# DSXiangLi/ChineseNER

Hardware: NVIDIA H100
Metric: sentences/sec bert_bilstm_crf MSRA L=128 (higher is better)
Workload: dtype bf16

## Files before the change

chinesener_b200/csrc/gemm_tc.cu:

```cuda
#include <stdlib.h>

#include <mutex>

#include "tc_common.cuh"

namespace {

using namespace tc;

constexpr int BM = 128;
constexpr int BK = 64;
constexpr int MMA_K = 16;
constexpr int NUM_MMA_WG = 2;
constexpr float kSkFixupCost = 10.0f;
constexpr int NUM_THREADS = 128 * (1 + NUM_MMA_WG);

constexpr int OUT_CHUNK_BYTES = 64 * 128;
constexpr int OUT_STAGE_BYTES = NUM_MMA_WG * 2 * OUT_CHUNK_BYTES;

template <int BN>
struct Cfg {
  static constexpr int STAGES = (BN == 256 || BN == 192) ? 4 : ((BN == 128) ? 6 : 8);
  static constexpr int A_BYTES = BM * BK * 2;
  static constexpr int B_BYTES = BN * BK * 2;
  static constexpr int RING_BYTES = STAGES * (A_BYTES + B_BYTES);
  static constexpr size_t SMEM = (size_t)RING_BYTES + OUT_STAGE_BYTES + 256;
  static_assert(SMEM <= 227 * 1024, "shared memory per block");
};

struct EpiArgs {
  const float* bias;
  const float* residual;
};

template <int EPI>
__host__ __device__ constexpr bool epi_f32() { return EPI == NER_EPI_F32 || EPI == NER_EPI_RES_F32 || EPI == NER_EPI_RES_RELU_F32; }

__device__ __forceinline__ float gelu_tanh(float x) {
  const float u = 0.7978845608028654f * fmaf(0.044715f * x * x, x, x);
  const float hx = 0.5f * x;
  return fmaf(hx, tanh_approx(u), hx);
}
__device__ __forceinline__ float gelu_erf(float x) { return 0.5f * x * (1.f + erff(x * 0.7071067811865476f)); }

__device__ __forceinline__ uint32_t pack_bf16x2(float a, float b) {
  __nv_bfloat162 v = __floats2bfloat162_rn(a, b);
  return *reinterpret_cast<uint32_t*>(&v);
}

struct SkArgs {
  float4* ws;
  int* flags;
};

struct SegIter {
  int num_kb, num_tiles, tile, stride;
  long long u, u1;
  bool sk;
  __device__ SegIter(bool sk_, int num_tiles_, int num_kb_, int id, int count)
      : num_kb(num_kb_), num_tiles(num_tiles_), sk(sk_) {
    if (sk) {
      const long long U = (long long)num_tiles * num_kb;
      u = (long long)id * U / count;
      u1 = (long long)(id + 1) * U / count;
    } else {
      tile = id;
      stride = count;
    }
  }
  __device__ bool next(int& t, int& kb0, int& kb1) {
    if (sk) {
      if (u >= u1) return false;
      t = (int)(u / num_kb);
      kb0 = (int)(u - (long long)t * num_kb);
      const long long rem = u1 - u;
      kb1 = (rem < (long long)(num_kb - kb0)) ? kb0 + (int)rem : num_kb;
      u += kb1 - kb0;
      return true;
    }
    if (tile >= num_tiles) return false;
    t = tile;
    kb0 = 0;
    kb1 = num_kb;
    tile += stride;
    return true;
  }
};

__device__ __forceinline__ int ld_acquire_gpu(const int* p) {
  int v;
  asm volatile("ld.acquire.gpu.global.s32 %0, [%1];" : "=r"(v) : "l"(p) : "memory");
  return v;
}
__device__ __forceinline__ void st_release_gpu(int* p, int v) {
  asm volatile("st.release.gpu.global.s32 [%0], %1;" ::"l"(p), "r"(v) : "memory");
}

__device__ __forceinline__ void mma_bar_sync() {
  asm volatile("bar.sync 1, %0;" ::"n"(128 * NUM_MMA_WG) : "memory");
}

template <int BN>
struct Ring {
  uint8_t* a;
  uint8_t* b;
  uint8_t* out;
  uint64_t* full;
  uint64_t* empty;
  __device__ Ring(uint8_t* smem) {
    using C = Cfg<BN>;
    a = smem;
    b = smem + C::STAGES * C::A_BYTES;
    out = smem + C::RING_BYTES;
    full = reinterpret_cast<uint64_t*>(out + OUT_STAGE_BYTES);
    empty = full + C::STAGES;
  }
};

struct RingPos {
  int stage = 0;
  uint32_t phase = 0;
  template <int STAGES>
  __device__ __forceinline__ void advance() {
    if (++stage == STAGES) {
      stage = 0;
      phase ^= 1u;
    }
  }
};

template <int BN, int STAGES, int CL, int TA, int TB, typename DA, typename DB>
__device__ __forceinline__ void mma_kblocks(float (&acc)[BN / 2], const Ring<BN>& ring, RingPos& pos, int kb0, int kb1,
                                            uint32_t a_off, DA desc_a, DB desc_b, const uint32_t (&empty_peer)[STAGES]) {
  const int lane = threadIdx.x & 31;
  int prev = -1;
  for (int kb = kb0; kb < kb1; ++kb) {
    mbar_wait(&ring.full[pos.stage], pos.phase);
    const uint32_t a_addr = smem_u32(ring.a + pos.stage * (BM * BK * 2)) + a_off;
    const uint32_t b_addr = smem_u32(ring.b + pos.stage * (BN * BK * 2));
    reg_fence(acc);
    wgmma_fence();
#pragma unroll
    for (int k = 0; k < BK / MMA_K; ++k)
      wgmma_bf16<BN, TA, TB>(acc, desc_a(a_addr, k), desc_b(b_addr, k), (kb > kb0 || k > 0) ? 1u : 0u);
    wgmma_commit();
    reg_fence(acc);
    if (prev >= 0) {
      wgmma_wait<1>();
      reg_fence(acc);
      if (lane == 0) {
        mbar_arrive(&ring.empty[prev]);
        if constexpr (CL == 2) mbar_arrive_cluster(empty_peer[prev]);
      }
    }
    prev = pos.stage;
    pos.template advance<STAGES>();
  }
  wgmma_wait<0>();
  reg_fence(acc);
  if (lane == 0 && prev >= 0) {
    mbar_arrive(&ring.empty[prev]);
    if constexpr (CL == 2) mbar_arrive_cluster(empty_peer[prev]);
  }
}

template <int EPI>
__device__ __forceinline__ float epi_act(float v) {
  if constexpr (EPI == NER_EPI_GELU_TANH_BF16) return gelu_tanh(v);
  else if constexpr (EPI == NER_EPI_GELU_ERF_BF16) return gelu_erf(v);
  else if constexpr (EPI == NER_EPI_RELU_BF16 || EPI == NER_EPI_RES_RELU_F32) return fmaxf(v, 0.f);
  else return v;
}

__device__ __forceinline__ void wg_bar_sync(int id) {
  asm volatile("bar.sync %0, 128;" ::"r"(id) : "memory");
}

template <int BN, int EPI>
__device__ __forceinline__ void epilogue_tma(const float (&acc)[BN / 2], const EpiArgs& ep, const CUtensorMap* tma_out,
                                             uint8_t* stage, uint32_t& buf, int row_wg, int n0, int M, int N) {
  constexpr bool F32 = epi_f32<EPI>();
  constexpr bool RES = EPI == NER_EPI_RES_F32 || EPI == NER_EPI_RES_RELU_F32;
  constexpr int CW = F32 ? 32 : 64;
  constexpr int JPC = CW / 8;
  const int t = threadIdx.x & 127, lane = t & 31, warp = t >> 5;
  const int bar = 1 + (threadIdx.x >> 7);
  const int r0 = 16 * warp + (lane >> 2);
  if (row_wg >= M) return;
#pragma unroll
  for (int c = 0; c < BN / CW; ++c) {
    const int col0 = n0 + c * CW;
    if (col0 >= N) break;
    uint8_t* sb = stage + buf * OUT_CHUNK_BYTES;
    if (t == 0) tma_store_wait_read<1>();
    wg_bar_sync(bar);
    float2 b[JPC];
#pragma unroll
    for (int jj = 0; jj < JPC; ++jj) {
      const int col = col0 + 8 * jj + 2 * (lane & 3);
      b[jj] = (ep.bias != nullptr && col < N) ? __ldg(reinterpret_cast<const float2*>(ep.bias + col)) : make_float2(0.f, 0.f);
    }
    if constexpr (F32) {
#pragma unroll
      for (int jj = 0; jj < JPC; ++jj) {
        const int j = c * JPC + jj, col = col0 + 8 * jj + 2 * (lane & 3);
#pragma unroll
        for (int h = 0; h < 2; ++h) {
          const int r = r0 + 8 * h;
          float v0 = acc[4 * j + 2 * h] + b[jj].x, v1 = acc[4 * j + 2 * h + 1] + b[jj].y;
          if constexpr (RES) {
            const int row = row_wg + r;
            if (row < M && col < N) {
              const float2 rv = *reinterpret_cast<const float2*>(ep.residual + (size_t)row * N + col);
              v0 += rv.x;
              v1 += rv.y;
            }
          }
          v0 = epi_act<EPI>(v0);
          v1 = epi_act<EPI>(v1);
          const int unit = (2 * jj + ((lane & 3) >> 1)) ^ (r & 7);
          *reinterpret_cast<float2*>(sb + r * 128 + unit * 16 + 8 * (lane & 1)) = make_float2(v0, v1);
        }
      }
    } else {
      const int i = lane >> 3, r = 16 * warp + 8 * (i & 1) + (lane & 7);
      const uint32_t row_addr = smem_u32(sb) + r * 128;
#pragma unroll
      for (int jj = 0; jj < JPC; jj += 2) {
        const int j = c * JPC + jj;
        uint32_t p[4];
#pragma unroll
        for (int q = 0; q < 4; ++q) {
          const int jq = j + (q >> 1), h = q & 1;
          const float2 bq = b[jj + (q >> 1)];
          p[q] = pack_bf16x2(epi_act<EPI>(acc[4 * jq + 2 * h] + bq.x), epi_act<EPI>(acc[4 * jq + 2 * h + 1] + bq.y));
        }
        stmatrix_x4(row_addr + (((jj + (i >> 1)) ^ (r & 7)) << 4), p[0], p[1], p[2], p[3]);
      }
    }
    fence_proxy_async();
    wg_bar_sync(bar);
    if (t == 0) {
      tma_store_2d(tma_out, sb, col0, row_wg);
      tma_store_commit();
    }
    buf ^= 1u;
  }
}

template <int BN>
__device__ __forceinline__ void epilogue_accumulate(const float (&acc)[BN / 2], float* dw, int row_w, int n0, int M,
                                                    int N) {
  const int lane = threadIdx.x & 31;
#pragma unroll
  for (int j = 0; j < BN / 8; ++j) {
    const int col = n0 + 8 * j + 2 * (lane & 3);
    if (col >= N) continue;
#pragma unroll
    for (int h = 0; h < 2; ++h) {
      const int row = row_w + (lane >> 2) + 8 * h;
      if (row >= M) continue;
      float2* p = reinterpret_cast<float2*>(dw + (size_t)row * N + col);
      const float2 r = *p;
      *p = make_float2(acc[4 * j + 2 * h] + 0.f + r.x, acc[4 * j + 2 * h + 1] + 0.f + r.y);
    }
  }
}

template <int BN, int CL>
__device__ __forceinline__ void init_ring(const Ring<BN>& ring) {
  if (threadIdx.x == 0) {
    for (int s = 0; s < Cfg<BN>::STAGES; ++s) {
      mbar_init(&ring.full[s], 1);
      mbar_init(&ring.empty[s], 4 * NUM_MMA_WG * CL);
    }
    fence_barrier_init();
  }
}

template <int BN, bool SK, int CL, int EPI>
__global__ void __launch_bounds__(NUM_THREADS, 1)
gemm_bf16_tc_kernel(const __grid_constant__ CUtensorMap tma_a, const __grid_constant__ CUtensorMap tma_b,
                    const __grid_constant__ CUtensorMap tma_out, EpiArgs ep, int M, int N, int K, SkArgs skargs) {
  using C = Cfg<BN>;
  constexpr int STAGES = C::STAGES;
  nerdev::pdl_launch_dependents();

  extern __shared__ __align__(1024) uint8_t smem_raw[];
  if ((smem_u32(smem_raw) & 1023u) != 0u) __trap();
  const Ring<BN> ring(smem_raw);

  const int wg = threadIdx.x >> 7;
  const uint32_t rank = CL == 2 ? cluster_ctarank() : 0u;
  const int id = CL == 2 ? (int)(blockIdx.x >> 1) : (int)blockIdx.x;
  const int count = CL == 2 ? (int)(gridDim.x >> 1) : (int)gridDim.x;

  const int num_m = (M + CL * BM - 1) / (CL * BM);
  const int num_n = (N + BN - 1) / BN;
  const int num_tiles = num_m * num_n;
  const int num_kb = (K + BK - 1) / BK;

  if (threadIdx.x == 0) {
    tma_prefetch_desc(&tma_a);
    tma_prefetch_desc(&tma_b);
    tma_prefetch_desc(&tma_out);
  }
  init_ring<BN, CL>(ring);
  if constexpr (CL == 2) cluster_sync_all();
  else __syncthreads();
  nerdev::pdl_wait();

  if (wg == 0) {
    setmaxnreg_dec<40>();
    if (threadIdx.x < 32 && elect_one()) {
      RingPos pos;
      SegIter it(SK, num_tiles, num_kb, id, count);
      int tile, kb0, kb1;
      while (it.next(tile, kb0, kb1)) {
        const int m_blk = tile / num_n, n_blk = tile - m_blk * num_n;
        const int row_a = (m_blk * CL + (int)rank) * BM;
        for (int kb = kb0; kb < kb1; ++kb) {
          mbar_wait(&ring.empty[pos.stage], pos.phase ^ 1u);
          mbar_arrive_expect_tx(&ring.full[pos.stage], C::A_BYTES + C::B_BYTES);
          tma_load_2d(ring.a + pos.stage * C::A_BYTES, &tma_a, &ring.full[pos.stage], kb * BK, row_a);
          if constexpr (CL == 2)
            tma_load_2d_mc(ring.b + pos.stage * C::B_BYTES + rank * (C::B_BYTES / 2), &tma_b, &ring.full[pos.stage],
                           kb * BK, n_blk * BN + (int)rank * (BN / 2), (uint16_t)0x3);
          else
            tma_load_2d(ring.b + pos.stage * C::B_BYTES, &tma_b, &ring.full[pos.stage], kb * BK, n_blk * BN);
          pos.advance<STAGES>();
        }
      }
    }
  } else {
    setmaxnreg_inc<232>();
    const int mw = wg - 1;
    const int ctid = threadIdx.x - 128;
    uint8_t* stage = ring.out + mw * 2 * OUT_CHUNK_BYTES;
    uint32_t buf = 0;
    uint32_t empty_peer[STAGES];
#pragma unroll
    for (int s = 0; s < STAGES; ++s) empty_peer[s] = CL == 2 ? mapa_u32(smem_u32(&ring.empty[s]), rank ^ 1u) : 0u;
    auto da = [](uint32_t addr, int k) { return make_wgmma_desc_sw128(addr + k * MMA_K * 2); };
    constexpr size_t SLOT = (size_t)BN * BM / 2;
    float2* ws = reinterpret_cast<float2*>(skargs.ws);
    RingPos pos;
    SegIter it(SK, num_tiles, num_kb, id, count);
    int tile, kb0, kb1;
    float acc[BN / 2];
    while (it.next(tile, kb0, kb1)) {
      const int m_blk = tile / num_n, n_blk = tile - m_blk * num_n;
      const int row0 = (m_blk * CL + (int)rank) * BM;
      mma_kblocks<BN, STAGES, CL, 0, 0>(acc, ring, pos, kb0, kb1, (uint32_t)(mw * 64 * BK * 2), da, da, empty_peer);
      if (SK && kb0 > 0) {
        float2* p = ws + (size_t)blockIdx.x * SLOT + ctid;
#pragma unroll
        for (int i = 0; i < BN / 4; ++i) __stcg(p + (size_t)i * 256, make_float2(acc[2 * i], acc[2 * i + 1]));
        __threadfence();
        mma_bar_sync();
        if (ctid == 0) st_release_gpu(skargs.flags + blockIdx.x, 1);
        continue;
      }
      int c_first = 0, n_part = 0;
      if (SK && kb1 < num_kb) {
        const long long U = (long long)num_tiles * num_kb, tile_end = (long long)(tile + 1) * num_kb;
        c_first = blockIdx.x + 1;
        for (int c = c_first; c < (int)gridDim.x; ++c) {
          const long long c0 = (long long)c * U / gridDim.x, c1 = (long long)(c + 1) * U / gridDim.x;
          if (c0 >= tile_end) break;
          if (c1 > c0) ++n_part; else if (n_part == 0) ++c_first;
        }
        if (ctid == 0) {
          for (int c = 0; c < n_part; ++c) {
            unsigned spins = 0;
            while (ld_acquire_gpu(skargs.flags + c_first + c) == 0)
              if (++spins > (1u << 28)) __trap();
          }
        }
        mma_bar_sync();
        __threadfence();
        for (int c = 0; c < n_part; ++c) {
          const float2* p = ws + (size_t)(c_first + c) * SLOT + ctid;
#pragma unroll
          for (int i = 0; i < BN / 4; ++i) {
            const float2 v = __ldcg(p + (size_t)i * 256);
            acc[2 * i] += v.x;
            acc[2 * i + 1] += v.y;
          }
        }
      }
      if constexpr (EPI == NER_EPI_DIAG_DISCARD) {
        if (M < 0) {
#pragma unroll
          for (int i = 0; i < BN / 2; ++i) reinterpret_cast<float*>(ring.a)[i * 256 + ctid] = acc[i];
        }
      } else {
        epilogue_tma<BN, EPI>(acc, ep, &tma_out, stage, buf, row0 + mw * 64, n_blk * BN, M, N);
      }
      if (n_part > 0) {
        mma_bar_sync();
        if (ctid < 32)
          for (int c = ctid; c < n_part; c += 32) skargs.flags[c_first + c] = 0;
      }
    }
    if ((threadIdx.x & 127) == 0) tma_store_wait_all();
  }
  if constexpr (CL == 2) cluster_sync_all();
}

constexpr int WG_MAXP = 6;
constexpr int WG_BN = 256;

struct WgradGroup {
  CUtensorMap a[WG_MAXP], b[WG_MAXP];
  float* dw[WG_MAXP];
  int m[WG_MAXP], n[WG_MAXP], b_col0[WG_MAXP];
  int tile_start[WG_MAXP + 1];
  int count, rows;
};

__global__ void __launch_bounds__(NUM_THREADS, 1)
gemm_wgrad_group_kernel(const __grid_constant__ WgradGroup grp) {
  constexpr int BN = WG_BN;
  using C = Cfg<BN>;
  constexpr int STAGES = C::STAGES;
  constexpr int BOX = 64 * 64 * 2;
  nerdev::pdl_launch_dependents();

  extern __shared__ __align__(1024) uint8_t smem_raw[];
  if ((smem_u32(smem_raw) & 1023u) != 0u) __trap();
  const Ring<BN> ring(smem_raw);

  const int wg = threadIdx.x >> 7;
  const int num_tiles = grp.tile_start[grp.count];
  const int num_kb = (grp.rows + BK - 1) / BK;

  init_ring<BN, 1>(ring);
  __syncthreads();
  nerdev::pdl_wait();

  auto locate = [&](int tile, int& p, int& m_blk, int& n_blk) {
    p = 0;
    while (p + 1 < grp.count && tile >= grp.tile_start[p + 1]) ++p;
    const int t = tile - grp.tile_start[p], num_n = grp.n[p] / BN;
    m_blk = t / num_n;
    n_blk = t - m_blk * num_n;
  };

  if (wg == 0) {
    setmaxnreg_dec<40>();
    if (threadIdx.x < 32 && elect_one()) {
      RingPos pos;
      for (int tile = blockIdx.x; tile < num_tiles; tile += gridDim.x) {
        int p, m_blk, n_blk;
        locate(tile, p, m_blk, n_blk);
        for (int kb = 0; kb < num_kb; ++kb) {
          mbar_wait(&ring.empty[pos.stage], pos.phase ^ 1u);
          mbar_arrive_expect_tx(&ring.full[pos.stage], C::A_BYTES + C::B_BYTES);
#pragma unroll
          for (int i = 0; i < BM / 64; ++i)
            tma_load_2d(ring.a + pos.stage * C::A_BYTES + i * BOX, &grp.a[p], &ring.full[pos.stage], m_blk * BM + i * 64, kb * BK);
#pragma unroll
          for (int i = 0; i < BN / 64; ++i)
            tma_load_2d(ring.b + pos.stage * C::B_BYTES + i * BOX, &grp.b[p], &ring.full[pos.stage],
                        grp.b_col0[p] + n_blk * BN + i * 64, kb * BK);
          pos.advance<STAGES>();
        }
      }
    }
  } else {
    setmaxnreg_inc<232>();
    const int mw = wg - 1;
    const int row_in_tile = mw * 64 + ((threadIdx.x >> 5) & 3) * 16;
    const uint32_t no_peer[STAGES] = {};
    auto da = [](uint32_t addr, int k) { return make_wgmma_desc_sw128(addr + k * 2048); };
    auto db = [](uint32_t addr, int k) { return make_wgmma_desc_sw128(addr + k * 2048, BOX); };
    RingPos pos;
    float acc[BN / 2];
    for (int tile = blockIdx.x; tile < num_tiles; tile += gridDim.x) {
      int p, m_blk, n_blk;
      locate(tile, p, m_blk, n_blk);
      mma_kblocks<BN, STAGES, 1, 1, 1>(acc, ring, pos, 0, num_kb, (uint32_t)(mw * BOX), da, db, no_peer);
      epilogue_accumulate<BN>(acc, grp.dw[p], m_blk * BM + row_in_tile, n_blk * BN, grp.m[p], grp.n[p]);
    }
  }
}

constexpr int FP8_BN = 128;
constexpr int FP8_BK = 128;
constexpr int FP8_MMA_K = 32;

template <int EPI>
__host__ __device__ constexpr bool epi_e4m3() { return EPI == NER_EPI_GELU_TANH_E4M3 || EPI == NER_EPI_GELU_ERF_E4M3; }

__device__ __forceinline__ void fp8_issue(float (&t)[FP8_BN / 2], const Ring<FP8_BN>& ring, int stage, uint32_t a_off) {
  const uint32_t a_addr = smem_u32(ring.a + stage * Cfg<FP8_BN>::A_BYTES) + a_off;
  const uint32_t b_addr = smem_u32(ring.b + stage * Cfg<FP8_BN>::B_BYTES);
  reg_fence(t);
  wgmma_fence();
#pragma unroll
  for (int k = 0; k < FP8_BK / FP8_MMA_K; ++k)
    wgmma_m64n128k32_e4m3(t, make_wgmma_desc_sw128(a_addr + k * FP8_MMA_K), make_wgmma_desc_sw128(b_addr + k * FP8_MMA_K),
                          k > 0 ? 1u : 0u);
  wgmma_commit();
  reg_fence(t);
}

__device__ __forceinline__ void fp8_promote(float (&acc)[FP8_BN / 2], const float (&t)[FP8_BN / 2], float s0, float s1) {
#pragma unroll
  for (int i = 0; i < FP8_BN / 2; ++i) acc[i] = fmaf(t[i], (i & 2) ? s1 : s0, acc[i]);
}

template <int EPI>
__device__ __forceinline__ void epilogue_e4m3(float (&acc)[FP8_BN / 2], const float* bias, float* out_scale,
                                              const CUtensorMap* tma_out, uint8_t* stage, uint32_t& buf, int row_wg, int n0,
                                              int M, int N) {
  const int t = threadIdx.x & 127, lane = t & 31, warp = t >> 5;
  const int bar = 1 + (threadIdx.x >> 7);
  const int r0 = 16 * warp + (lane >> 2);
  if (row_wg >= M) return;
  uint8_t* sb = stage + buf * OUT_CHUNK_BYTES;
  if (t == 0) tma_store_wait_read<1>();
  wg_bar_sync(bar);
  float amax[2] = {0.f, 0.f};
#pragma unroll
  for (int j = 0; j < FP8_BN / 8; ++j) {
    const int col = n0 + 8 * j + 2 * (lane & 3);
    const float2 b = bias != nullptr ? __ldg(reinterpret_cast<const float2*>(bias + col)) : make_float2(0.f, 0.f);
#pragma unroll
    for (int h = 0; h < 2; ++h) {
#pragma unroll
      for (int c = 0; c < 2; ++c) {
        const float x = acc[4 * j + 2 * h + c] + (c ? b.y : b.x);
        float v;
        if constexpr (EPI == NER_EPI_GELU_ERF_E4M3) v = gelu_erf(x);
        else v = 0.5f * x * (1.f + tanhf(0.7978845608028654f * fmaf(0.044715f * x * x, x, x)));
        acc[4 * j + 2 * h + c] = v;
        amax[h] = fmaxf(amax[h], fabsf(v));
      }
    }
  }
  float inv[2];
#pragma unroll
  for (int h = 0; h < 2; ++h) {
    amax[h] = fmaxf(amax[h], __shfl_xor_sync(0xffffffffu, amax[h], 1));
    amax[h] = fmaxf(amax[h], __shfl_xor_sync(0xffffffffu, amax[h], 2));
    const float s = nerdev::e4m3_scale(amax[h]);
    inv[h] = __frcp_rn(s);
    const int row = row_wg + r0 + 8 * h;
    if ((lane & 3) == 0 && row < M) out_scale[(size_t)row * (N / FP8_BN) + n0 / FP8_BN] = s;
  }
#pragma unroll
  for (int j = 0; j < FP8_BN / 8; ++j) {
#pragma unroll
    for (int h = 0; h < 2; ++h) {
      const int r = r0 + 8 * h;
      const uint16_t q = nerdev::cvt_e4m3x2(acc[4 * j + 2 * h] * inv[h], acc[4 * j + 2 * h + 1] * inv[h]);
      *reinterpret_cast<uint16_t*>(sb + r * 128 + (((j >> 1) ^ (r & 7)) << 4) + 8 * (j & 1) + 2 * (lane & 3)) = q;
    }
  }
  fence_proxy_async();
  wg_bar_sync(bar);
  if (t == 0) {
    tma_store_2d(tma_out, sb, n0, row_wg);
    tma_store_commit();
  }
  buf ^= 1u;
}

template <int EPI>
__global__ void __launch_bounds__(NUM_THREADS, 1)
gemm_e4m3_tc_kernel(const __grid_constant__ CUtensorMap tma_a, const __grid_constant__ CUtensorMap tma_b,
                    const __grid_constant__ CUtensorMap tma_out, const float* __restrict__ a_scale,
                    const float* __restrict__ w_scale, const float* __restrict__ bias, float* __restrict__ out_scale, int M,
                    int N, int K) {
  using C = Cfg<FP8_BN>;
  constexpr int STAGES = C::STAGES;
  nerdev::pdl_launch_dependents();

  extern __shared__ __align__(1024) uint8_t smem_raw[];
  if ((smem_u32(smem_raw) & 1023u) != 0u) __trap();
  const Ring<FP8_BN> ring(smem_raw);

  const int wg = threadIdx.x >> 7;
  const int num_n = N / FP8_BN;
  const int num_tiles = ((M + BM - 1) / BM) * num_n;
  const int num_kb = K / FP8_BK;

  if (threadIdx.x == 0) {
    tma_prefetch_desc(&tma_a);
    tma_prefetch_desc(&tma_b);
    tma_prefetch_desc(&tma_out);
  }
  init_ring<FP8_BN, 1>(ring);
  __syncthreads();
  nerdev::pdl_wait();

  if (wg == 0) {
    setmaxnreg_dec<40>();
    if (threadIdx.x < 32 && elect_one()) {
      RingPos pos;
      for (int tile = blockIdx.x; tile < num_tiles; tile += gridDim.x) {
        const int m_blk = tile / num_n, n_blk = tile - m_blk * num_n;
        for (int kb = 0; kb < num_kb; ++kb) {
          mbar_wait(&ring.empty[pos.stage], pos.phase ^ 1u);
          mbar_arrive_expect_tx(&ring.full[pos.stage], C::A_BYTES + C::B_BYTES);
          tma_load_2d(ring.a + pos.stage * C::A_BYTES, &tma_a, &ring.full[pos.stage], kb * FP8_BK, m_blk * BM);
          tma_load_2d(ring.b + pos.stage * C::B_BYTES, &tma_b, &ring.full[pos.stage], kb * FP8_BK, n_blk * FP8_BN);
          pos.advance<STAGES>();
        }
      }
    }
  } else {
    setmaxnreg_inc<232>();
    const int mw = wg - 1;
    const int lane = threadIdx.x & 31, warp = (threadIdx.x >> 5) & 3;
    uint8_t* stage = ring.out + mw * 2 * OUT_CHUNK_BYTES;
    uint32_t buf = 0;
    const uint32_t a_off = (uint32_t)(mw * 64 * FP8_BK);
    RingPos pos;
    float acc[FP8_BN / 2], tmp[FP8_BN / 2];
    for (int tile = blockIdx.x; tile < num_tiles; tile += gridDim.x) {
      const int m_blk = tile / num_n, n_blk = tile - m_blk * num_n;
      const int row_wg = m_blk * BM + mw * 64, n0 = n_blk * FP8_BN;
      const int ra = row_wg + 16 * warp + (lane >> 2);
      const float* sa0 = a_scale + (size_t)min(ra, M - 1) * num_kb;
      const float* sa1 = a_scale + (size_t)min(ra + 8, M - 1) * num_kb;
#pragma unroll
      for (int i = 0; i < FP8_BN / 2; ++i) acc[i] = 0.f;
      for (int kb = 0; kb < num_kb; ++kb) {
        const float s0 = __ldg(sa0 + kb), s1 = __ldg(sa1 + kb);
        mbar_wait(&ring.full[pos.stage], pos.phase);
        fp8_issue(tmp, ring, pos.stage, a_off);
        wgmma_wait<0>();
        reg_fence(tmp);
        if (lane == 0) mbar_arrive(&ring.empty[pos.stage]);
        fp8_promote(acc, tmp, s0, s1);
        pos.advance<STAGES>();
      }
#pragma unroll
      for (int j = 0; j < FP8_BN / 8; ++j) {
        const float2 sw = __ldg(reinterpret_cast<const float2*>(w_scale + n0 + 8 * j + 2 * (lane & 3)));
        acc[4 * j] *= sw.x;
        acc[4 * j + 1] *= sw.y;
        acc[4 * j + 2] *= sw.x;
        acc[4 * j + 3] *= sw.y;
      }
      if constexpr (epi_e4m3<EPI>())
        epilogue_e4m3<EPI>(acc, bias, out_scale, &tma_out, stage, buf, row_wg, n0, M, N);
      else
        epilogue_tma<FP8_BN, NER_EPI_BF16>(acc, EpiArgs{bias, nullptr}, &tma_out, stage, buf, row_wg, n0, M, N);
    }
    if ((threadIdx.x & 127) == 0) tma_store_wait_all();
  }
}

int make_map_2d(CUtensorMap* map, const void* ptr, uint64_t rows, uint64_t cols, uint32_t box_rows, bool f32 = false) {
  EncodeTiledFn fn = tensor_map_encode_fn();
  if (fn == nullptr) return NER_ERR_NO_DRIVER;
  const uint32_t esz = f32 ? 4 : 2;
  cuuint64_t dims[2] = {cols, rows};
  cuuint64_t strides[1] = {cols * esz};
  cuuint32_t box[2] = {128 / esz, box_rows};
  cuuint32_t estr[2] = {1, 1};
  CUresult r = fn(map, f32 ? CU_TENSOR_MAP_DATA_TYPE_FLOAT32 : CU_TENSOR_MAP_DATA_TYPE_BFLOAT16, 2, const_cast<void*>(ptr),
                  dims, strides, box, estr, CU_TENSOR_MAP_INTERLEAVE_NONE, CU_TENSOR_MAP_SWIZZLE_128B,
                  CU_TENSOR_MAP_L2_PROMOTION_L2_256B, CU_TENSOR_MAP_FLOAT_OOB_FILL_NONE);
  return r == CUDA_SUCCESS ? NER_OK : NER_ERR_INVALID_ARG;
}

int gemm_auto_policy() {
  static int v = -1;
  if (v < 0) {
    const char* e = getenv("NER_GEMM_POLICY");
    v = e ? atoi(e) : 0;
  }
  return v;
}

int sm_count() { return ner_num_sms(); }

struct SkScratch {
  int dev;
  cudaStream_t st;
  float4* ws;
  int* flags;
};
constexpr int kMaxSkScratch = 16;
SkScratch g_sk[kMaxSkScratch];
int g_sk_n = 0;
std::mutex g_sk_mu;

bool sk_scratch(cudaStream_t st, SkArgs* out) {
  int dev = 0;
  if (cudaGetDevice(&dev) != cudaSuccess) return false;
  std::lock_guard<std::mutex> lk(g_sk_mu);
  for (int i = 0; i < g_sk_n; ++i)
    if (g_sk[i].dev == dev && g_sk[i].st == st) {
      out->ws = g_sk[i].ws;
      out->flags = g_sk[i].flags;
      return true;
    }
  if (g_sk_n == kMaxSkScratch) return false;
  cudaStreamCaptureStatus cap = cudaStreamCaptureStatusNone;
  if (cudaStreamIsCapturing(st, &cap) != cudaSuccess || cap != cudaStreamCaptureStatusNone) {
    (void)cudaGetLastError();
    return false;
  }
  const size_t slot = (size_t)(256 / 32) * 8 * 128 * sizeof(float4);
  float4* ws = nullptr;
  int* flags = nullptr;
  if (cudaMalloc(&ws, slot * sm_count()) != cudaSuccess) {
    (void)cudaGetLastError();
    return false;
  }
  if (cudaMalloc(&flags, sizeof(int) * sm_count()) != cudaSuccess || cudaMemset(flags, 0, sizeof(int) * sm_count()) != cudaSuccess) {
    (void)cudaGetLastError();
    cudaFree(ws);
    return false;
  }
  cudaDeviceSynchronize();
  g_sk[g_sk_n++] = SkScratch{dev, st, ws, flags};
  out->ws = ws;
  out->flags = flags;
  return true;
}

template <typename... KArgs, typename... Args>
cudaError_t launch_ex(void (*kern)(KArgs...), int grid, size_t smem, cudaStream_t st, int cl, Args... args) {
  cudaError_t e = cudaFuncSetAttribute(kern, cudaFuncAttributeMaxDynamicSharedMemorySize, (int)smem);
  if (e != cudaSuccess) return e;
  cudaLaunchConfig_t cfg{};
  cfg.gridDim = dim3(grid);
  cfg.blockDim = dim3(NUM_THREADS);
  cfg.dynamicSmemBytes = smem;
  cfg.stream = st;
  cudaLaunchAttribute attr[2];
  attr[0].id = cudaLaunchAttributeProgrammaticStreamSerialization;
  attr[0].val.programmaticStreamSerializationAllowed = 1;
  attr[1].id = cudaLaunchAttributeClusterDimension;
  attr[1].val.clusterDim.x = cl;
  attr[1].val.clusterDim.y = 1;
  attr[1].val.clusterDim.z = 1;
  cfg.attrs = attr;
  cfg.numAttrs = 2;
  return cudaLaunchKernelEx(&cfg, kern, static_cast<KArgs>(args)...);
}

template <int BN, int CL, int EPI>
int launch_gemm(const void* A, const void* Wt, EpiArgs ep, void* out, int M, int N, int K, cudaStream_t st, bool sk) {
  CUtensorMap ma, mb, mo;
  int rc = make_map_2d(&ma, A, (uint64_t)M, (uint64_t)K, BM);
  if (rc != NER_OK) return rc;
  rc = make_map_2d(&mb, Wt, (uint64_t)N, (uint64_t)K, BN / CL);
  if (rc != NER_OK) return rc;
  rc = make_map_2d(&mo, out, (uint64_t)M, (uint64_t)N, 64, epi_f32<EPI>());
  if (rc != NER_OK) return rc;
  const size_t smem = Cfg<BN>::SMEM;
  const int tiles = ((M + CL * BM - 1) / (CL * BM)) * ((N + BN - 1) / BN);
  const int num_kb = (K + BK - 1) / BK;
  SkArgs ska{nullptr, nullptr};
  cudaError_t e;
  if constexpr (CL == 1) {
    if constexpr ((BN == 256 || BN == 128) && EPI != NER_EPI_DIAG_DISCARD) {
      if (sk && (long long)tiles * num_kb >= sm_count() && sk_scratch(st, &ska)) {
        e = launch_ex(gemm_bf16_tc_kernel<BN, true, 1, EPI>, sm_count(), smem, st, 1, ma, mb, mo, ep, M, N, K, ska);
        if (e != cudaSuccess) return NER_ERR_CUDA_BASE - (int)e;
        return ner_launch_status();
      }
    }
    e = launch_ex(gemm_bf16_tc_kernel<BN, false, 1, EPI>, tiles < sm_count() ? tiles : sm_count(), smem, st, 1, ma, mb, mo,
                  ep, M, N, K, ska);
  } else {
    const int max_pairs = sm_count() / 2;
    const int pairs = tiles < max_pairs ? tiles : max_pairs;
    e = launch_ex(gemm_bf16_tc_kernel<BN, false, 2, EPI>, 2 * pairs, smem, st, 2, ma, mb, mo, ep, M, N, K, ska);
  }
  if (e != cudaSuccess) return NER_ERR_CUDA_BASE - (int)e;
  return ner_launch_status();
}

template <int BN, int CL>
int launch_gemm(const void* A, const void* Wt, EpiArgs ep, void* out, int M, int N, int K, int epilogue, cudaStream_t st,
                bool sk = false) {
  switch (epilogue) {
    case NER_EPI_F32: return launch_gemm<BN, CL, NER_EPI_F32>(A, Wt, ep, out, M, N, K, st, sk);
    case NER_EPI_BF16: return launch_gemm<BN, CL, NER_EPI_BF16>(A, Wt, ep, out, M, N, K, st, sk);
    case NER_EPI_GELU_TANH_BF16: return launch_gemm<BN, CL, NER_EPI_GELU_TANH_BF16>(A, Wt, ep, out, M, N, K, st, sk);
    case NER_EPI_GELU_ERF_BF16: return launch_gemm<BN, CL, NER_EPI_GELU_ERF_BF16>(A, Wt, ep, out, M, N, K, st, sk);
    case NER_EPI_RELU_BF16: return launch_gemm<BN, CL, NER_EPI_RELU_BF16>(A, Wt, ep, out, M, N, K, st, sk);
    case NER_EPI_RES_F32: return launch_gemm<BN, CL, NER_EPI_RES_F32>(A, Wt, ep, out, M, N, K, st, sk);
    case NER_EPI_RES_RELU_F32: return launch_gemm<BN, CL, NER_EPI_RES_RELU_F32>(A, Wt, ep, out, M, N, K, st, sk);
    case NER_EPI_DIAG_DISCARD: return launch_gemm<BN, CL, NER_EPI_DIAG_DISCARD>(A, Wt, ep, out, M, N, K, st, sk);
    default: return NER_ERR_INVALID_ARG;
  }
}

}

static int make_map_bf16_box64(CUtensorMap* map, const void* ptr, uint64_t rows, uint64_t cols) {
  return make_map_2d(map, ptr, rows, cols, 64);
}

extern "C" int ner_wgrad_group_bf16(const ner_wgrad_problem* problems_host, int count, int rows, ner_stream_t stream) {
  if (count < 0 || rows < 0 || (count > 0 && !problems_host)) return NER_ERR_INVALID_ARG;
  if (count == 0 || rows == 0) return NER_OK;
  if (count > WG_MAXP) return NER_ERR_UNSUPPORTED;
  WgradGroup g;
  g.count = count;
  g.rows = rows;
  g.tile_start[0] = 0;
  for (int p = 0; p < count; ++p) {
    const ner_wgrad_problem& q = problems_host[p];
    if (!q.x_bf16 || !q.dy_bf16 || !q.dw || q.k_in < 1 || q.n_out < 1 || q.ld_x < q.k_in || q.dy_col0 < 0 ||
        q.ld_dy < q.dy_col0 + q.n_out)
      return NER_ERR_INVALID_ARG;
    if (q.k_in % BM != 0 || q.n_out % WG_BN != 0 || q.ld_x % 8 != 0 || q.ld_dy % 8 != 0 || q.dy_col0 % 64 != 0)
      return NER_ERR_UNSUPPORTED;
    if ((reinterpret_cast<uintptr_t>(q.x_bf16) & 15) || (reinterpret_cast<uintptr_t>(q.dy_bf16) & 15) ||
        (reinterpret_cast<uintptr_t>(q.dw) & 15))
      return NER_ERR_INVALID_ARG;
    int rc = make_map_bf16_box64(&g.a[p], q.x_bf16, (uint64_t)rows, (uint64_t)q.ld_x);
    if (rc != NER_OK) return rc;
    rc = make_map_bf16_box64(&g.b[p], q.dy_bf16, (uint64_t)rows, (uint64_t)q.ld_dy);
    if (rc != NER_OK) return rc;
    g.dw[p] = q.dw;
    g.m[p] = q.k_in;
    g.n[p] = q.n_out;
    g.b_col0[p] = q.dy_col0;
    g.tile_start[p + 1] = g.tile_start[p] + (q.k_in / BM) * (q.n_out / WG_BN);
  }
  for (int p = count; p < WG_MAXP; ++p) {
    g.a[p] = g.a[0]; g.b[p] = g.b[0];
    g.dw[p] = nullptr; g.m[p] = g.n[p] = g.b_col0[p] = 0;
    g.tile_start[p + 1] = g.tile_start[count];
  }
  const int tiles = g.tile_start[count];
  const int grid = tiles < sm_count() ? tiles : sm_count();
  cudaError_t e = launch_ex(gemm_wgrad_group_kernel, grid, Cfg<WG_BN>::SMEM, static_cast<cudaStream_t>(stream), 1, g);
  if (e != cudaSuccess) return NER_ERR_CUDA_BASE - (int)e;
  return ner_launch_status();
}

extern "C" int ner_gemm_bf16(const void* A, const void* Wt, const float* bias, const float* residual, void* out,
                             int M, int N, int K, int epilogue, int tile_n, ner_stream_t stream) {
  if (M < 0 || N < 1 || K < 1) return NER_ERR_INVALID_ARG;
  if (M == 0) return NER_OK;
  if (!A || !Wt || !out) return NER_ERR_INVALID_ARG;
  if ((epilogue < NER_EPI_F32 || epilogue > NER_EPI_RES_RELU_F32) && epilogue != NER_EPI_DIAG_DISCARD) return NER_ERR_INVALID_ARG;
  if ((epilogue == NER_EPI_RES_F32 || epilogue == NER_EPI_RES_RELU_F32) && !residual) return NER_ERR_INVALID_ARG;
  if ((K % 8) != 0 || (N % 32) != 0) return NER_ERR_UNSUPPORTED;
  if ((reinterpret_cast<uintptr_t>(A) & 15) || (reinterpret_cast<uintptr_t>(Wt) & 15) ||
      (reinterpret_cast<uintptr_t>(out) & 15))
    return NER_ERR_INVALID_ARG;
  if ((reinterpret_cast<uintptr_t>(bias) & 7) || (reinterpret_cast<uintptr_t>(residual) & 7)) return NER_ERR_INVALID_ARG;
  EpiArgs ep{bias, residual};
  cudaStream_t st = static_cast<cudaStream_t>(stream);
  int bn = tile_n;
  bool sk = false;
  if (bn == NER_TILE_SK_256 || bn == NER_TILE_SK_128) {
    sk = true;
    bn = (bn == NER_TILE_SK_256) ? 256 : 128;
  } else if (bn == NER_TILE_AUTO_THROUGHPUT || (bn == 0 && gemm_auto_policy() == 1)) {
    bn = (N % 256 == 0) ? 256 : (N % 192 == 0) ? 192 : 128;
  }
  if (bn == 0) {
    const int mt = (M + BM - 1) / BM, sms = sm_count(), num_kb = (K + BK - 1) / BK;
    const int cand[3] = {256, 192, 128};
    const float cost[3] = {1.00f, 0.80f, 0.64f};
    float best = 1e30f;
    bn = 128;
    for (int i = 0; i < 3; ++i) {
      if (N % cand[i] != 0) continue;
      const int tiles = mt * (N / cand[i]);
      const float t = (float)((tiles + sms - 1) / sms) * cost[i] * (float)num_kb;
      if (t < best - 1e-6f) {
        best = t;
        bn = cand[i];
      }
    }
    if (N % 256 == 0) {
      const long long units = (long long)mt * (N / 256) * num_kb;
      const float t_sk = (float)((units + sms - 1) / sms) + kSkFixupCost;
      if (units >= sms && t_sk < 0.9f * best) {
        sk = true;
        bn = 256;
      }
    }
  }
  switch (bn) {
    case 256: return launch_gemm<256, 1>(A, Wt, ep, out, M, N, K, epilogue, st, sk);
    case 192: return launch_gemm<192, 1>(A, Wt, ep, out, M, N, K, epilogue, st);
    case 128: return launch_gemm<128, 1>(A, Wt, ep, out, M, N, K, epilogue, st, sk);
    case 64: return launch_gemm<64, 1>(A, Wt, ep, out, M, N, K, epilogue, st);
    case NER_TILE_2CTA_256: return launch_gemm<256, 2>(A, Wt, ep, out, M, N, K, epilogue, st);
    case NER_TILE_2CTA_128: return launch_gemm<128, 2>(A, Wt, ep, out, M, N, K, epilogue, st);
    default: return NER_ERR_INVALID_ARG;
  }
}

namespace {
int make_map_e4m3(CUtensorMap* map, const void* ptr, uint64_t rows, uint64_t cols, uint32_t box_rows) {
  EncodeTiledFn fn = tensor_map_encode_fn();
  if (fn == nullptr) return NER_ERR_NO_DRIVER;
  cuuint64_t dims[2] = {cols, rows};
  cuuint64_t strides[1] = {cols};
  cuuint32_t box[2] = {128, box_rows};
  cuuint32_t estr[2] = {1, 1};
  CUresult r = fn(map, CU_TENSOR_MAP_DATA_TYPE_UINT8, 2, const_cast<void*>(ptr), dims, strides, box, estr,
                  CU_TENSOR_MAP_INTERLEAVE_NONE, CU_TENSOR_MAP_SWIZZLE_128B, CU_TENSOR_MAP_L2_PROMOTION_L2_256B,
                  CU_TENSOR_MAP_FLOAT_OOB_FILL_NONE);
  return r == CUDA_SUCCESS ? NER_OK : NER_ERR_INVALID_ARG;
}

template <int EPI>
int launch_gemm_e4m3(const void* A, const float* a_scale, const void* Wt, const float* w_scale, const float* bias, void* out,
                     float* out_scale, int M, int N, int K, cudaStream_t st) {
  CUtensorMap ma, mb, mo;
  int rc = make_map_e4m3(&ma, A, (uint64_t)M, (uint64_t)K, BM);
  if (rc != NER_OK) return rc;
  rc = make_map_e4m3(&mb, Wt, (uint64_t)N, (uint64_t)K, FP8_BN);
  if (rc != NER_OK) return rc;
  rc = epi_e4m3<EPI>() ? make_map_e4m3(&mo, out, (uint64_t)M, (uint64_t)N, 64) : make_map_2d(&mo, out, (uint64_t)M, (uint64_t)N, 64);
  if (rc != NER_OK) return rc;
  const int tiles = ((M + BM - 1) / BM) * (N / FP8_BN);
  const cudaError_t e = launch_ex(gemm_e4m3_tc_kernel<EPI>, tiles < sm_count() ? tiles : sm_count(), Cfg<FP8_BN>::SMEM, st, 1,
                                  ma, mb, mo, a_scale, w_scale, bias, out_scale, M, N, K);
  if (e != cudaSuccess) return NER_ERR_CUDA_BASE - (int)e;
  return ner_launch_status();
}
}

extern "C" int ner_gemm_e4m3(const void* A, const float* a_scale, const void* Wt, const float* w_scale, const float* bias,
                             void* out, float* out_scale, int M, int N, int K, int epilogue, ner_stream_t stream) {
  if (M < 0 || N < 1 || K < 1) return NER_ERR_INVALID_ARG;
  if (epilogue != NER_EPI_BF16 && epilogue != NER_EPI_GELU_TANH_E4M3 && epilogue != NER_EPI_GELU_ERF_E4M3)
    return NER_ERR_INVALID_ARG;
  if (K % FP8_BK != 0 || N % FP8_BN != 0) return NER_ERR_UNSUPPORTED;
  if (M == 0) return NER_OK;
  const bool q_out = epilogue != NER_EPI_BF16;
  if (!A || !a_scale || !Wt || !w_scale || !out || (q_out && !out_scale)) return NER_ERR_INVALID_ARG;
  if ((reinterpret_cast<uintptr_t>(A) & 15) || (reinterpret_cast<uintptr_t>(Wt) & 15) || (reinterpret_cast<uintptr_t>(out) & 15))
    return NER_ERR_INVALID_ARG;
  if ((reinterpret_cast<uintptr_t>(w_scale) & 7) || (reinterpret_cast<uintptr_t>(bias) & 7)) return NER_ERR_INVALID_ARG;
  cudaStream_t st = static_cast<cudaStream_t>(stream);
  switch (epilogue) {
    case NER_EPI_BF16: return launch_gemm_e4m3<NER_EPI_BF16>(A, a_scale, Wt, w_scale, bias, out, out_scale, M, N, K, st);
    case NER_EPI_GELU_TANH_E4M3:
      return launch_gemm_e4m3<NER_EPI_GELU_TANH_E4M3>(A, a_scale, Wt, w_scale, bias, out, out_scale, M, N, K, st);
    default: return launch_gemm_e4m3<NER_EPI_GELU_ERF_E4M3>(A, a_scale, Wt, w_scale, bias, out, out_scale, M, N, K, st);
  }
}
```

Before: 49420.

## Replace 2-CTA cluster GEMM with ping-pong consumer kernel over paired CTAs

Replaces the cluster-of-two cooperative GEMM path with a new ping-pong kernel. Each CTA loads 64 rows of A, and B is multicast across the pair. The two MMA warpgroups alternate whole tiles, using named barriers so one warpgroup's epilogue overlaps the other's mainloop. The grid is sized from the occupancy query for active clusters. The auto-throughput policy now falls back to the cost-model tile picker when there are at least as many tiles as SMs. The 2-CTA path only runs when it is explicitly requested, and the policy tweak applies only to the auto-throughput mode.

```diff
diff --git a/chinesener_b200/csrc/gemm_tc.cu b/chinesener_b200/csrc/gemm_tc.cu
--- a/chinesener_b200/csrc/gemm_tc.cu
+++ b/chinesener_b200/csrc/gemm_tc.cu
@@ -18,10 +18,10 @@
 constexpr int OUT_CHUNK_BYTES = 64 * 128;
 constexpr int OUT_STAGE_BYTES = NUM_MMA_WG * 2 * OUT_CHUNK_BYTES;
 
-template <int BN>
+template <int BN, int AROWS = BM>
 struct Cfg {
-  static constexpr int STAGES = (BN == 256 || BN == 192) ? 4 : ((BN == 128) ? 6 : 8);
-  static constexpr int A_BYTES = BM * BK * 2;
+  static constexpr int STAGES = AROWS == BM ? ((BN == 256 || BN == 192) ? 4 : ((BN == 128) ? 6 : 8)) : (BN == 256 ? 4 : 8);
+  static constexpr int A_BYTES = AROWS * BK * 2;
   static constexpr int B_BYTES = BN * BK * 2;
   static constexpr int RING_BYTES = STAGES * (A_BYTES + B_BYTES);
   static constexpr size_t SMEM = (size_t)RING_BYTES + OUT_STAGE_BYTES + 256;
@@ -100,7 +100,7 @@
   asm volatile("bar.sync 1, %0;" ::"n"(128 * NUM_MMA_WG) : "memory");
 }
 
-template <int BN>
+template <int BN, int AROWS = BM>
 struct Ring {
   uint8_t* a;
   uint8_t* b;
@@ -108,7 +108,7 @@
   uint64_t* full;
   uint64_t* empty;
   __device__ Ring(uint8_t* smem) {
-    using C = Cfg<BN>;
+    using C = Cfg<BN, AROWS>;
     a = smem;
     b = smem + C::STAGES * C::A_BYTES;
     out = smem + C::RING_BYTES;
@@ -129,14 +129,14 @@
   }
 };
 
-template <int BN, int STAGES, int CL, int TA, int TB, typename DA, typename DB>
-__device__ __forceinline__ void mma_kblocks(float (&acc)[BN / 2], const Ring<BN>& ring, RingPos& pos, int kb0, int kb1,
-                                            uint32_t a_off, DA desc_a, DB desc_b, const uint32_t (&empty_peer)[STAGES]) {
+template <int BN, int STAGES, int CL, int TA, int TB, int AROWS, typename DA, typename DB>
+__device__ __forceinline__ void mma_kblocks(float (&acc)[BN / 2], const Ring<BN, AROWS>& ring, RingPos& pos, int kb0, int kb1,
+                                            uint32_t a_off, DA desc_a, DB desc_b, uint32_t empty_peer) {
   const int lane = threadIdx.x & 31;
   int prev = -1;
   for (int kb = kb0; kb < kb1; ++kb) {
     mbar_wait(&ring.full[pos.stage], pos.phase);
-    const uint32_t a_addr = smem_u32(ring.a + pos.stage * (BM * BK * 2)) + a_off;
+    const uint32_t a_addr = smem_u32(ring.a + pos.stage * (AROWS * BK * 2)) + a_off;
     const uint32_t b_addr = smem_u32(ring.b + pos.stage * (BN * BK * 2));
     reg_fence(acc);
     wgmma_fence();
@@ -150,7 +150,7 @@
       reg_fence(acc);
       if (lane == 0) {
         mbar_arrive(&ring.empty[prev]);
-        if constexpr (CL == 2) mbar_arrive_cluster(empty_peer[prev]);
+        if constexpr (CL == 2) mbar_arrive_cluster(empty_peer + 8u * prev);
       }
     }
     prev = pos.stage;
@@ -160,7 +160,7 @@
   reg_fence(acc);
   if (lane == 0 && prev >= 0) {
     mbar_arrive(&ring.empty[prev]);
-    if constexpr (CL == 2) mbar_arrive_cluster(empty_peer[prev]);
+    if constexpr (CL == 2) mbar_arrive_cluster(empty_peer + 8u * prev);
   }
 }
 
@@ -267,18 +267,18 @@
   }
 }
 
-template <int BN, int CL>
-__device__ __forceinline__ void init_ring(const Ring<BN>& ring) {
+template <int BN, int CL, int WARPS = 4 * NUM_MMA_WG, int AROWS = BM>
+__device__ __forceinline__ void init_ring(const Ring<BN, AROWS>& ring) {
   if (threadIdx.x == 0) {
-    for (int s = 0; s < Cfg<BN>::STAGES; ++s) {
+    for (int s = 0; s < Cfg<BN, AROWS>::STAGES; ++s) {
       mbar_init(&ring.full[s], 1);
-      mbar_init(&ring.empty[s], 4 * NUM_MMA_WG * CL);
+      mbar_init(&ring.empty[s], WARPS * CL);
     }
     fence_barrier_init();
   }
 }
 
-template <int BN, bool SK, int CL, int EPI>
+template <int BN, bool SK, int EPI>
 __global__ void __launch_bounds__(NUM_THREADS, 1)
 gemm_bf16_tc_kernel(const __grid_constant__ CUtensorMap tma_a, const __grid_constant__ CUtensorMap tma_b,
                     const __grid_constant__ CUtensorMap tma_out, EpiArgs ep, int M, int N, int K, SkArgs skargs) {
@@ -291,11 +291,7 @@
   const Ring<BN> ring(smem_raw);
 
   const int wg = threadIdx.x >> 7;
-  const uint32_t rank = CL == 2 ? cluster_ctarank() : 0u;
-  const int id = CL == 2 ? (int)(blockIdx.x >> 1) : (int)blockIdx.x;
-  const int count = CL == 2 ? (int)(gridDim.x >> 1) : (int)gridDim.x;
-
-  const int num_m = (M + CL * BM - 1) / (CL * BM);
+  const int num_m = (M + BM - 1) / BM;
   const int num_n = (N + BN - 1) / BN;
   const int num_tiles = num_m * num_n;
   const int num_kb = (K + BK - 1) / BK;
@@ -305,29 +301,23 @@
     tma_prefetch_desc(&tma_b);
     tma_prefetch_desc(&tma_out);
   }
-  init_ring<BN, CL>(ring);
-  if constexpr (CL == 2) cluster_sync_all();
-  else __syncthreads();
+  init_ring<BN, 1>(ring);
+  __syncthreads();
   nerdev::pdl_wait();
 
   if (wg == 0) {
     setmaxnreg_dec<40>();
     if (threadIdx.x < 32 && elect_one()) {
       RingPos pos;
-      SegIter it(SK, num_tiles, num_kb, id, count);
+      SegIter it(SK, num_tiles, num_kb, blockIdx.x, gridDim.x);
       int tile, kb0, kb1;
       while (it.next(tile, kb0, kb1)) {
         const int m_blk = tile / num_n, n_blk = tile - m_blk * num_n;
-        const int row_a = (m_blk * CL + (int)rank) * BM;
         for (int kb = kb0; kb < kb1; ++kb) {
           mbar_wait(&ring.empty[pos.stage], pos.phase ^ 1u);
           mbar_arrive_expect_tx(&ring.full[pos.stage], C::A_BYTES + C::B_BYTES);
-          tma_load_2d(ring.a + pos.stage * C::A_BYTES, &tma_a, &ring.full[pos.stage], kb * BK, row_a);
-          if constexpr (CL == 2)
-            tma_load_2d_mc(ring.b + pos.stage * C::B_BYTES + rank * (C::B_BYTES / 2), &tma_b, &ring.full[pos.stage],
-                           kb * BK, n_blk * BN + (int)rank * (BN / 2), (uint16_t)0x3);
-          else
-            tma_load_2d(ring.b + pos.stage * C::B_BYTES, &tma_b, &ring.full[pos.stage], kb * BK, n_blk * BN);
+          tma_load_2d(ring.a + pos.stage * C::A_BYTES, &tma_a, &ring.full[pos.stage], kb * BK, m_blk * BM);
+          tma_load_2d(ring.b + pos.stage * C::B_BYTES, &tma_b, &ring.full[pos.stage], kb * BK, n_blk * BN);
           pos.advance<STAGES>();
         }
       }
@@ -338,20 +328,17 @@
     const int ctid = threadIdx.x - 128;
     uint8_t* stage = ring.out + mw * 2 * OUT_CHUNK_BYTES;
     uint32_t buf = 0;
-    uint32_t empty_peer[STAGES];
-#pragma unroll
-    for (int s = 0; s < STAGES; ++s) empty_peer[s] = CL == 2 ? mapa_u32(smem_u32(&ring.empty[s]), rank ^ 1u) : 0u;
     auto da = [](uint32_t addr, int k) { return make_wgmma_desc_sw128(addr + k * MMA_K * 2); };
     constexpr size_t SLOT = (size_t)BN * BM / 2;
     float2* ws = reinterpret_cast<float2*>(skargs.ws);
     RingPos pos;
-    SegIter it(SK, num_tiles, num_kb, id, count);
+    SegIter it(SK, num_tiles, num_kb, blockIdx.x, gridDim.x);
     int tile, kb0, kb1;
     float acc[BN / 2];
     while (it.next(tile, kb0, kb1)) {
       const int m_blk = tile / num_n, n_blk = tile - m_blk * num_n;
-      const int row0 = (m_blk * CL + (int)rank) * BM;
-      mma_kblocks<BN, STAGES, CL, 0, 0>(acc, ring, pos, kb0, kb1, (uint32_t)(mw * 64 * BK * 2), da, da, empty_peer);
+      const int row0 = m_blk * BM;
+      mma_kblocks<BN, STAGES, 1, 0, 0>(acc, ring, pos, kb0, kb1, (uint32_t)(mw * 64 * BK * 2), da, da, 0u);
       if (SK && kb0 > 0) {
         float2* p = ws + (size_t)blockIdx.x * SLOT + ctid;
 #pragma unroll
@@ -405,7 +392,88 @@
     }
     if ((threadIdx.x & 127) == 0) tma_store_wait_all();
   }
-  if constexpr (CL == 2) cluster_sync_all();
+}
+
+constexpr int PP_ROWS = 64;
+constexpr int PP_BAR = 4;
+
+template <int BN, int EPI>
+__global__ void __launch_bounds__(NUM_THREADS, 1)
+gemm_bf16_tc_pingpong_kernel(const __grid_constant__ CUtensorMap tma_a, const __grid_constant__ CUtensorMap tma_b,
+                          const __grid_constant__ CUtensorMap tma_out, EpiArgs ep, int M, int N, int K) {
+  using C = Cfg<BN, PP_ROWS>;
+  constexpr int STAGES = C::STAGES;
+  nerdev::pdl_launch_dependents();
+
+  extern __shared__ __align__(1024) uint8_t smem_raw[];
+  if ((smem_u32(smem_raw) & 1023u) != 0u) __trap();
+  const Ring<BN, PP_ROWS> ring(smem_raw);
+
+  const int wg = threadIdx.x >> 7;
+  const uint32_t rank = cluster_ctarank();
+  const int cid = (int)(blockIdx.x >> 1), G = (int)(gridDim.x >> 1);
+  const int num_n = (N + BN - 1) / BN;
+  const int num_tiles = ((M + BM - 1) / BM) * num_n;
+  const int num_kb = (K + BK - 1) / BK;
+  const int my_tiles = cid < num_tiles ? (num_tiles - cid + G - 1) / G : 0;
+
+  if (threadIdx.x == 0) {
+    tma_prefetch_desc(&tma_a);
+    tma_prefetch_desc(&tma_b);
+    tma_prefetch_desc(&tma_out);
+  }
+  init_ring<BN, 2, 4>(ring);
+  cluster_sync_all();
+  nerdev::pdl_wait();
+
+  if (wg == 0) {
+    setmaxnreg_dec<40>();
+    if (threadIdx.x < 32 && elect_one()) {
+      RingPos pos;
+      for (int i = 0; i < my_tiles; ++i) {
+        const int tile = cid + i * G;
+        const int m_blk = tile / num_n, n_blk = tile - m_blk * num_n;
+        for (int kb = 0; kb < num_kb; ++kb) {
+          mbar_wait(&ring.empty[pos.stage], pos.phase ^ 1u);
+          mbar_arrive_expect_tx(&ring.full[pos.stage], C::A_BYTES + C::B_BYTES);
+          tma_load_2d(ring.a + pos.stage * C::A_BYTES, &tma_a, &ring.full[pos.stage], kb * BK,
+                      m_blk * BM + (int)rank * PP_ROWS);
+          tma_load_2d_mc(ring.b + pos.stage * C::B_BYTES + rank * (C::B_BYTES / 2), &tma_b, &ring.full[pos.stage],
+                         kb * BK, n_blk * BN + (int)rank * (BN / 2), (uint16_t)0x3);
+          pos.advance<STAGES>();
+        }
+      }
+    }
+  } else {
+    setmaxnreg_inc<232>();
+    const int mw = wg - 1;
+    uint8_t* stage = ring.out + mw * 2 * OUT_CHUNK_BYTES;
+    uint32_t buf = 0;
+    const uint32_t empty_peer = mapa_u32(smem_u32(ring.empty), rank ^ 1u);
+    auto da = [](uint32_t addr, int k) { return make_wgmma_desc_sw128(addr + k * MMA_K * 2); };
+    float acc[BN / 2];
+    for (int i = mw; i < my_tiles; i += 2) {
+      const int tile = cid + i * G;
+      const int m_blk = tile / num_n, n_blk = tile - m_blk * num_n;
+      const long long p0 = (long long)i * num_kb;
+      RingPos pos;
+      pos.stage = (int)(p0 % STAGES);
+      pos.phase = (uint32_t)((p0 / STAGES) & 1);
+      if (i > 0) asm volatile("bar.sync %0, 256;" ::"r"(PP_BAR + mw) : "memory");
+      mma_kblocks<BN, STAGES, 2, 0, 0>(acc, ring, pos, 0, num_kb, 0u, da, da, empty_peer);
+      if (i + 1 < my_tiles) asm volatile("bar.arrive %0, 256;" ::"r"(PP_BAR + (mw ^ 1)) : "memory");
+      if constexpr (EPI == NER_EPI_DIAG_DISCARD) {
+        if (M < 0) {
+#pragma unroll
+          for (int j = 0; j < BN / 2; ++j) reinterpret_cast<float*>(ring.a)[j * 256 + threadIdx.x - 128] = acc[j];
+        }
+      } else {
+        epilogue_tma<BN, EPI>(acc, ep, &tma_out, stage, buf, m_blk * BM + (int)rank * PP_ROWS, n_blk * BN, M, N);
+      }
+    }
+    if ((threadIdx.x & 127) == 0) tma_store_wait_all();
+  }
+  cluster_sync_all();
 }
 
 constexpr int WG_MAXP = 6;
@@ -472,7 +540,6 @@
     setmaxnreg_inc<232>();
     const int mw = wg - 1;
     const int row_in_tile = mw * 64 + ((threadIdx.x >> 5) & 3) * 16;
-    const uint32_t no_peer[STAGES] = {};
     auto da = [](uint32_t addr, int k) { return make_wgmma_desc_sw128(addr + k * 2048); };
     auto db = [](uint32_t addr, int k) { return make_wgmma_desc_sw128(addr + k * 2048, BOX); };
     RingPos pos;
@@ -480,7 +547,7 @@
     for (int tile = blockIdx.x; tile < num_tiles; tile += gridDim.x) {
       int p, m_blk, n_blk;
       locate(tile, p, m_blk, n_blk);
-      mma_kblocks<BN, STAGES, 1, 1, 1>(acc, ring, pos, 0, num_kb, (uint32_t)(mw * BOX), da, db, no_peer);
+      mma_kblocks<BN, STAGES, 1, 1, 1>(acc, ring, pos, 0, num_kb, (uint32_t)(mw * BOX), da, db, 0u);
       epilogue_accumulate<BN>(acc, grp.dw[p], m_blk * BM + row_in_tile, n_blk * BN, grp.m[p], grp.n[p]);
     }
   }
@@ -747,51 +814,81 @@
   return cudaLaunchKernelEx(&cfg, kern, static_cast<KArgs>(args)...);
 }
 
-template <int BN, int CL, int EPI>
+template <int BN, int EPI>
+int max_pair_clusters() {
+  static int n = -1;
+  if (n < 0) {
+    auto kern = gemm_bf16_tc_pingpong_kernel<BN, EPI>;
+    constexpr size_t smem = Cfg<BN, PP_ROWS>::SMEM;
+    int v = 0;
+    cudaLaunchConfig_t cfg{};
+    cfg.gridDim = dim3(2);
+    cfg.blockDim = dim3(NUM_THREADS);
+    cfg.dynamicSmemBytes = smem;
+    cudaLaunchAttribute attr[1];
+    attr[0].id = cudaLaunchAttributeClusterDimension;
+    attr[0].val.clusterDim.x = 2;
+    attr[0].val.clusterDim.y = 1;
+    attr[0].val.clusterDim.z = 1;
+    cfg.attrs = attr;
+    cfg.numAttrs = 1;
+    if (cudaFuncSetAttribute(kern, cudaFuncAttributeMaxDynamicSharedMemorySize, (int)smem) != cudaSuccess ||
+        cudaOccupancyMaxActiveClusters(&v, kern, &cfg) != cudaSuccess)
+      v = 0;
+    (void)cudaGetLastError();
+    n = v;
+  }
+  return n;
+}
+
+template <int BN, bool PAIR, int EPI>
 int launch_gemm(const void* A, const void* Wt, EpiArgs ep, void* out, int M, int N, int K, cudaStream_t st, bool sk) {
   CUtensorMap ma, mb, mo;
-  int rc = make_map_2d(&ma, A, (uint64_t)M, (uint64_t)K, BM);
+  int rc = make_map_2d(&ma, A, (uint64_t)M, (uint64_t)K, PAIR ? PP_ROWS : BM);
   if (rc != NER_OK) return rc;
-  rc = make_map_2d(&mb, Wt, (uint64_t)N, (uint64_t)K, BN / CL);
+  rc = make_map_2d(&mb, Wt, (uint64_t)N, (uint64_t)K, PAIR ? BN / 2 : BN);
   if (rc != NER_OK) return rc;
   rc = make_map_2d(&mo, out, (uint64_t)M, (uint64_t)N, 64, epi_f32<EPI>());
   if (rc != NER_OK) return rc;
-  const size_t smem = Cfg<BN>::SMEM;
-  const int tiles = ((M + CL * BM - 1) / (CL * BM)) * ((N + BN - 1) / BN);
+  const int tiles = ((M + BM - 1) / BM) * ((N + BN - 1) / BN);
   const int num_kb = (K + BK - 1) / BK;
-  SkArgs ska{nullptr, nullptr};
   cudaError_t e;
-  if constexpr (CL == 1) {
+  if constexpr (PAIR) {
+    static_assert(BN == 128 || BN == 256, "ping-pong tiles");
+    const int max_cl = max_pair_clusters<BN, EPI>();
+    if (max_cl < 1) return NER_ERR_UNSUPPORTED;
+    const int per_cluster = (tiles + max_cl - 1) / max_cl;
+    const int clusters = (tiles + per_cluster - 1) / per_cluster;
+    e = launch_ex(gemm_bf16_tc_pingpong_kernel<BN, EPI>, 2 * clusters, Cfg<BN, PP_ROWS>::SMEM, st, 2, ma, mb, mo, ep, M, N, K);
+  } else {
+    constexpr size_t smem = Cfg<BN>::SMEM;
+    SkArgs ska{nullptr, nullptr};
     if constexpr ((BN == 256 || BN == 128) && EPI != NER_EPI_DIAG_DISCARD) {
       if (sk && (long long)tiles * num_kb >= sm_count() && sk_scratch(st, &ska)) {
-        e = launch_ex(gemm_bf16_tc_kernel<BN, true, 1, EPI>, sm_count(), smem, st, 1, ma, mb, mo, ep, M, N, K, ska);
+        e = launch_ex(gemm_bf16_tc_kernel<BN, true, EPI>, sm_count(), smem, st, 1, ma, mb, mo, ep, M, N, K, ska);
         if (e != cudaSuccess) return NER_ERR_CUDA_BASE - (int)e;
         return ner_launch_status();
       }
     }
-    e = launch_ex(gemm_bf16_tc_kernel<BN, false, 1, EPI>, tiles < sm_count() ? tiles : sm_count(), smem, st, 1, ma, mb, mo,
-                  ep, M, N, K, ska);
-  } else {
-    const int max_pairs = sm_count() / 2;
-    const int pairs = tiles < max_pairs ? tiles : max_pairs;
-    e = launch_ex(gemm_bf16_tc_kernel<BN, false, 2, EPI>, 2 * pairs, smem, st, 2, ma, mb, mo, ep, M, N, K, ska);
+    e = launch_ex(gemm_bf16_tc_kernel<BN, false, EPI>, tiles < sm_count() ? tiles : sm_count(), smem, st, 1, ma, mb, mo, ep,
+                  M, N, K, ska);
   }
   if (e != cudaSuccess) return NER_ERR_CUDA_BASE - (int)e;
   return ner_launch_status();
 }
 
-template <int BN, int CL>
+template <int BN, bool PAIR>
 int launch_gemm(const void* A, const void* Wt, EpiArgs ep, void* out, int M, int N, int K, int epilogue, cudaStream_t st,
                 bool sk = false) {
   switch (epilogue) {
-    case NER_EPI_F32: return launch_gemm<BN, CL, NER_EPI_F32>(A, Wt, ep, out, M, N, K, st, sk);
-    case NER_EPI_BF16: return launch_gemm<BN, CL, NER_EPI_BF16>(A, Wt, ep, out, M, N, K, st, sk);
-    case NER_EPI_GELU_TANH_BF16: return launch_gemm<BN, CL, NER_EPI_GELU_TANH_BF16>(A, Wt, ep, out, M, N, K, st, sk);
-    case NER_EPI_GELU_ERF_BF16: return launch_gemm<BN, CL, NER_EPI_GELU_ERF_BF16>(A, Wt, ep, out, M, N, K, st, sk);
-    case NER_EPI_RELU_BF16: return launch_gemm<BN, CL, NER_EPI_RELU_BF16>(A, Wt, ep, out, M, N, K, st, sk);
-    case NER_EPI_RES_F32: return launch_gemm<BN, CL, NER_EPI_RES_F32>(A, Wt, ep, out, M, N, K, st, sk);
-    case NER_EPI_RES_RELU_F32: return launch_gemm<BN, CL, NER_EPI_RES_RELU_F32>(A, Wt, ep, out, M, N, K, st, sk);
-    case NER_EPI_DIAG_DISCARD: return launch_gemm<BN, CL, NER_EPI_DIAG_DISCARD>(A, Wt, ep, out, M, N, K, st, sk);
+    case NER_EPI_F32: return launch_gemm<BN, PAIR, NER_EPI_F32>(A, Wt, ep, out, M, N, K, st, sk);
+    case NER_EPI_BF16: return launch_gemm<BN, PAIR, NER_EPI_BF16>(A, Wt, ep, out, M, N, K, st, sk);
+    case NER_EPI_GELU_TANH_BF16: return launch_gemm<BN, PAIR, NER_EPI_GELU_TANH_BF16>(A, Wt, ep, out, M, N, K, st, sk);
+    case NER_EPI_GELU_ERF_BF16: return launch_gemm<BN, PAIR, NER_EPI_GELU_ERF_BF16>(A, Wt, ep, out, M, N, K, st, sk);
+    case NER_EPI_RELU_BF16: return launch_gemm<BN, PAIR, NER_EPI_RELU_BF16>(A, Wt, ep, out, M, N, K, st, sk);
+    case NER_EPI_RES_F32: return launch_gemm<BN, PAIR, NER_EPI_RES_F32>(A, Wt, ep, out, M, N, K, st, sk);
+    case NER_EPI_RES_RELU_F32: return launch_gemm<BN, PAIR, NER_EPI_RES_RELU_F32>(A, Wt, ep, out, M, N, K, st, sk);
+    case NER_EPI_DIAG_DISCARD: return launch_gemm<BN, PAIR, NER_EPI_DIAG_DISCARD>(A, Wt, ep, out, M, N, K, st, sk);
     default: return NER_ERR_INVALID_ARG;
   }
 }
@@ -863,6 +960,7 @@
     bn = (bn == NER_TILE_SK_256) ? 256 : 128;
   } else if (bn == NER_TILE_AUTO_THROUGHPUT || (bn == 0 && gemm_auto_policy() == 1)) {
     bn = (N % 256 == 0) ? 256 : (N % 192 == 0) ? 192 : 128;
+    if (tile_n == NER_TILE_AUTO_THROUGHPUT && (long long)((M + BM - 1) / BM) * ((N + bn - 1) / bn) >= sm_count()) bn = 0;
   }
   if (bn == 0) {
     const int mt = (M + BM - 1) / BM, sms = sm_count(), num_kb = (K + BK - 1) / BK;
@@ -889,12 +987,12 @@
     }
   }
   switch (bn) {
-    case 256: return launch_gemm<256, 1>(A, Wt, ep, out, M, N, K, epilogue, st, sk);
-    case 192: return launch_gemm<192, 1>(A, Wt, ep, out, M, N, K, epilogue, st);
-    case 128: return launch_gemm<128, 1>(A, Wt, ep, out, M, N, K, epilogue, st, sk);
-    case 64: return launch_gemm<64, 1>(A, Wt, ep, out, M, N, K, epilogue, st);
-    case NER_TILE_2CTA_256: return launch_gemm<256, 2>(A, Wt, ep, out, M, N, K, epilogue, st);
-    case NER_TILE_2CTA_128: return launch_gemm<128, 2>(A, Wt, ep, out, M, N, K, epilogue, st);
+    case 256: return launch_gemm<256, false>(A, Wt, ep, out, M, N, K, epilogue, st, sk);
+    case 192: return launch_gemm<192, false>(A, Wt, ep, out, M, N, K, epilogue, st);
+    case 128: return launch_gemm<128, false>(A, Wt, ep, out, M, N, K, epilogue, st, sk);
+    case 64: return launch_gemm<64, false>(A, Wt, ep, out, M, N, K, epilogue, st);
+    case NER_TILE_2CTA_256: return launch_gemm<256, true>(A, Wt, ep, out, M, N, K, epilogue, st);
+    case NER_TILE_2CTA_128: return launch_gemm<128, true>(A, Wt, ep, out, M, N, K, epilogue, st);
     default: return NER_ERR_INVALID_ARG;
   }
 }
```

New measurement: 50040 (median of 6 runs). 1.3% higher.
